# USNavalResearchLaboratory/mgen

Measured on AMD Instinct MI355X. Metric: device-resident MgenMsg pack+unpack GB/s and Mmsg/s at 1/2/4/8 MI355X, higher is better.
Workload: dtype u8; 1 GPU; udp_unpack_crc_1M_x_1024B; records_per_gpu=1048576, record_bytes=1024, checksum=True, output=mgenx_rec rows (32 B), parallelism=flow-sharded x1 (independent slabs)

## Files before the change

mgen_amd/csrc/mgenx_unpack.hip:

```cpp
#include <type_traits>

#include "mgenx_kernels.hpp"
#include "mgenx_parse.hpp"

namespace mgenx {

constexpr int kUnpackThreads = 1024;
constexpr int kRep = 32;
constexpr int kRepDwords = 4 * 256 * kRep;
constexpr int kSmallTabDwords = 1024;
constexpr int kFoldTabs = 6;
constexpr size_t kUnpackLdsBytes = (size_t)(kRepDwords + kFoldTabs * kSmallTabDwords) * 4u;


__device__ __forceinline__ uint32_t a64_s1(uint32_t lane) { return ((lane & 31u) << 2) | (1u << 16); }

typedef __attribute__((address_space(3))) uint32_t lds_u32_t;
__device__ __forceinline__ uint32_t lds_u32(const uint8_t*, uint32_t addr, uint32_t imm) {
  return *(const lds_u32_t*)(addr + imm);
}

__device__ __forceinline__ uint32_t xor3(uint32_t a, uint32_t b, uint32_t c) {
  return __builtin_amdgcn_bitop3_b32(a, b, c, 0x96);
}
// ... 1055 lines not shown
      st_g8_nt(at(u8b, 1), r.o[4]);
      return;
    }
    st_g32(at(u32, 4), r.o[0]);
    st_g32(at((uint64_t)c.dst_addr4, 4), r.o[1]);
    st_g16(at(u16, 2), r.o[2]);
    st_g8(at(u8a, 1), r.o[3]);
    st_g8(at(u8b, 1), r.o[4]);
  };
  auto decide = [&](const u32x4_t& pf, bool live) {
    const uint32_t w0 = prefix_word(pf, 0);
    const uint32_t w5 = prefix_word(pf, 5);
    const bool v2 = ((w0 >> 16) & 0xffu) == 2u;
    const bool flagged = force || ((((w0 >> 24) & MGENX_FLAG_CHECKSUM) != 0) && v2);
    const uint32_t t = (w5 >> 16) & 0xffu;
    return live && flagged && (tcp || (v2 && (t == 1u || t == 2u)));
  };

  u32x4_t pf;
  auto load_group = [&](uint32_t gg) {
    const uint32_t i = rec_idx(gg);
    const uint32_t boff = base_off(is_live(i), i);
    if (!kAligned) pf = ld_hdr(boff);
#pragma unroll
    for (int j = 0; j < NR; j++) {
      d[j] = ld_row(boff, j);
      __builtin_amdgcn_sched_barrier(0);
    }
  };
  load_group(g);
  table_writes(lds, tab_regs);
  asm volatile("s_waitcnt lgkmcnt(0)" ::: "memory");
  __builtin_amdgcn_s_barrier();
  if (g >= g_end) return;
  bool first = true;
  while (g < g_end) {
    uint32_t idx = rec_idx(g);
    bool live = is_live(idx);
    if (!first) {
      const uint32_t boff = base_off(live, idx);
      if (!kAligned) pf = ld_hdr(boff);
#pragma unroll
      for (int j = 0; j < NR; j++) {
        d[j] = ld_row(boff, j);
        __builtin_amdgcn_sched_barrier(0);
      }
    }
    first = false;
    auto step = [&](const u32x4_t& pf_cur, u32x4_t& pf_nxt) {
      const uint32_t gn = g + n_waves;
      const bool has_next = gn < g_end;
      const uint32_t idx_n = rec_idx(has_next ? gn : g);
      const bool live_n = has_next && is_live(idx_n);
      const uint32_t boff_n = base_off(live_n, idx_n);
      if (!kAligned) pf_nxt = ld_hdr(boff_n);
      asm volatile("" ::: "memory");
      const u32x4_t hdr = kAligned ? d[0] : pf_cur;
      const bool needs_crc = decide(hdr, live);
      const bool any = __any(needs_crc);
      Out early;
      if (kAligned && !kAblNoTail) early = decode(hdr, idx, live);

      uint32_t ha[4] = {0u, 0u, 0u, 0u}, hb[4] = {0u, 0u, 0u, 0u};
#pragma unroll
      for (int j = 0; j < NR - 1; j++) {
        u32x4_t x = d[j];
        if (j == 0) {
          const int s0 = -pos0;
          if (s0 > 0) {
            const u32x4_t zero = {0u, 0u, 0u, 0u};
            x = s0 < 16 ? shl_bytes(x, s0) : zero;
          }
        }
        const uint32_t xw[4] = {x.x, x.y, x.z, x.w};
        uint32_t c4[4];
#pragma unroll
        for (int b = 0; b < 4; b++) {
          if (kAblXor)
            c4[b] = (ha[b] << 1) ^ xw[b];
          else
            c4[b] = xor3(ha[b], hb[b], xw[b]);
        }
        __builtin_amdgcn_sched_barrier(0);
        d[j] = ld_row(boff_n, j);
        __builtin_amdgcn_sched_barrier(0);
        if (kAblXor) {
#pragma unroll
          for (int b = 0; b < 4; b++) ha[b] = c4[b];
          continue;
        }
#pragma unroll
        for (int b = 0; b < 4; b++) a64_parts(ldsb, c4[b], s1, ha[b], hb[b]);
      }
      const u32x4_t xf = d[NR - 1];
      uint32_t f0 = xor3(ha[0], hb[0], xf.x), f1 = xor3(ha[1], hb[1], xf.y);
      uint32_t f2 = xor3(ha[2], hb[2], xf.z);
      uint32_t f3 = xor3(ha[3], hb[3], q == 3 ? bswap32(xf.w) : xf.w);
      asm volatile("" : "+v"(f0), "+v"(f1), "+v"(f2), "+v"(f3));
      __builtin_amdgcn_sched_barrier(0);
      d[NR - 1] = ld_row(boff_n, NR - 1);
      __builtin_amdgcn_sched_barrier(0);
      const uint32_t v = shift_tab(fold + 3 * 1024, f0) ^ shift_tab(fold + 2 * 1024, f1) ^
                         shift_tab(fold + 1 * 1024, f2) ^ shift_tab(fold, f3);
      const uint32_t* lt = fold + (q == 0 ? 5 : (q == 1 ? 4 : 3)) * 1024;
      uint32_t s = (q == 3) ? v : shift_tab(lt, v);
      s ^= __shfl_xor(s, 1);
      s ^= __shfl_xor(s, 2);
      if (kAblNoTail) {
        if (s == 0x9E3779B9u && lane == 0) p.cols.err[idx] = (uint8_t)needs_crc;
      } else {
        const Out r = kAligned ? early : decode(hdr, idx, live);
        emit(r, idx, needs_crc && s != expect);
      }
      asm volatile("" ::"v"(boff_n + (uint32_t)(pos0 + 64)));
      g = gn;
      idx = idx_n;
      live = live_n;
      return has_next && any;
    };
    u32x4_t pf2;
    if (kAligned) {
      while (step(pf, pf2)) {
      }
    } else {
      for (;;) {
        if (!step(pf, pf2)) break;
        if (!step(pf2, pf)) break;
      }
    }
    for (; g < g_end; g += n_waves) {
      const uint32_t i = rec_idx(g);
      const bool lv = is_live(i);
      const u32x4_t ph = ld_hdr(base_off(lv, i));
      const bool nc = decide(ph, lv);
      if (__any(nc)) break;
      emit(decode(ph, i, lv), i, false);
    }
  }
  if (kAblBurst) {
    uint32_t k = 0;
    for (uint32_t gg = wave_id; gg < g_end; gg += n_waves, k++) {
      const uint32_t i = rec_idx(gg);
      const uint64_t seq = (uint64_t)wave_id * 8192u + k * 512u + 8u * (uint32_t)lane;
      const uint64_t a = (uint64_t)p.cols.rows + (kAblBurstSeq ? seq : (uint64_t)i * 32 + 8 * q);
      if (i < p.n) {
        if (kAblWt) st_g64_wt(a, (uint64_t)gg);
        else if (kAblAltStore) st_g64(a, (uint64_t)gg);
        else st_g64_nt(a, (uint64_t)gg);
      }
    }
  }
}

template <int NR, int RS = 4, int K = 16>
__global__ void __launch_bounds__(kUnpackThreads)
unpack_fixed_ring_kernel(UnpackParams p, uint32_t expect) {
  static_assert(NR == 8 || NR == 16, "ring kernel: 512- or 1024-byte records");
  static_assert(NR % RS == 0, "the ring divides the record's rows");
  extern __shared__ __attribute__((aligned(16))) uint32_t lds[];
  const uint32_t* fold = lds + kRepDwords;
  const uint8_t* ldsb = reinterpret_cast<const uint8_t*>(lds);
  const TableRegs tab_regs = table_loads(p.tabs);
  asm volatile("" ::: "memory");

  const int lane = threadIdx.x & 63;
  const int q = lane & 3;
  const uint32_t s1 = a64_s1((uint32_t)lane);
  const uint32_t wave_id = __builtin_amdgcn_readfirstlane(
      blockIdx.x * (blockDim.x >> 6) + (threadIdx.x >> 6));
  const uint32_t n_waves = gridDim.x * (blockDim.x >> 6);
  const uint32_t g_end = (p.n + 15u) >> 4;
  const bool force = (p.opts & MGENX_OPT_CHECKSUM_FORCE) != 0;
  const bool tcp = (p.opts & MGENX_OPT_TCP) != 0;
  const uint32_t L = p.fixed_len;

  auto rec_idx = [&](uint32_t gg) { return (gg << 4) + (uint32_t)(lane >> 2); };
  auto is_live = [&](uint32_t i) {
    const uint64_t off = (uint64_t)i * p.stride;
    return i < p.n && off <= p.slab_bytes && L <= p.slab_bytes - off;
  };
  auto row_base = [&](uint32_t gg) {
    const uint32_t i = rec_idx(gg);
    return (is_live(i) ? i * (uint32_t)p.stride : 64u) + 16u * (uint32_t)q;
  };
  auto ld = [&](uint32_t base, int j) { return ldu128(p.slab + (uint64_t)base + 64 * j); };
  auto decide = [&](const u32x4_t& pf, bool live) {
    const uint32_t w0 = prefix_word(pf, 0);
    const uint32_t w5 = prefix_word(pf, 5);
    const bool v2 = ((w0 >> 16) & 0xffu) == 2u;
    const bool flagged = force || ((((w0 >> 24) & MGENX_FLAG_CHECKSUM) != 0) && v2);
    const uint32_t t = (w5 >> 16) & 0xffu;
    return live && flagged && (tcp || (v2 && (t == 1u || t == 2u)));
  };
  auto decode = [&](const u32x4_t& pf, uint32_t idx, bool live, uint32_t& o0, uint32_t& o1) {
    uint32_t w[8];
#pragma unroll
    for (int j = 0; j < 8; j++) w[j] = prefix_word(pf, j);
    const uint32_t w10 = prefix_word(pf, 10);
    const uint32_t D = w[5] >> 24;
    const uint32_t hw = (D == 4u) ? w[7] : w10;
    const uint32_t gi = (28u + D + (hw >> 24)) >> 2;
    const uint32_t g3 = (prefix_word(pf, 11) & (0u - (uint32_t)(gi == 8u))) |
                        (prefix_word(pf, 12) & (0u - (uint32_t)(gi == 9u))) |
                        (prefix_word(pf, 14) & (0u - (uint32_t)(gi == 11u))) |
                        (prefix_word(pf, 15) & (0u - (uint32_t)(gi == 12u)));
    uint32_t flow = bswap32(w[1]), seq = bswap32(w[2]), sec = bswap32(w[3]);
    uint32_t usec = bswap32(w[4]), dst4 = w[6];
    uint32_t msg_len = bswap16((uint16_t)(w[0] & 0xffffu));
    uint32_t dport = bswap16((uint16_t)(w[5] & 0xffffu));
    const uint32_t hlen = 44u + D + (hw >> 24);
    uint32_t plen = bswap16((uint16_t)(g3 >> 16));
    if (!(plen != 0 && hlen + plen <= L)) plen = 0;
    uint32_t flags = w[0] >> 24, err = 0, dtype = (w[5] >> 16) & 0xffu, dlen = D;
    uint32_t ptype = (g3 >> 8) & 0xffu, gps = g3 & 0xffu;
    const bool slow = live && !fast_layout(w[0], w[5], hw);
    if (__any(slow)) {
      Hdr h;
      if (slow && q == 0) parse_header(p.slab + (uint64_t)idx * p.stride, L, false, w, h);
      auto bc = [&](uint32_t& dst, uint32_t v) {
        v = (uint32_t)__builtin_amdgcn_mov_dpp((int)v, 0x00, 0xf, 0xf, false);
        if (slow) dst = v;
      };
      bc(flow, h.flow); bc(seq, h.seq); bc(sec, h.sec); bc(usec, h.usec); bc(dst4, h.dst4);
      bc(msg_len, h.msg_len); bc(dport, h.dst_port); bc(plen, h.plen); bc(flags, h.flags);
      bc(err, h.err); bc(dtype, h.dst_type); bc(dlen, h.dst_len); bc(ptype, h.ptype);
      bc(gps, h.gps);
    }
    if (!live) {
      flow = seq = sec = usec = dst4 = msg_len = dport = plen = flags = dtype = dlen = 0;
      ptype = gps = 0;
      err = MGENX_ERROR_OOB;
    }
    o0 = q == 0 ? flow : q == 1 ? sec : q == 2 ? dst4 : (plen | flags << 16 | err << 24);
    o1 = q == 0 ? seq : q == 1 ? usec : q == 2 ? (msg_len | dport << 16)
                                              : (dtype | dlen << 8 | ptype << 16 | gps << 24);
  };
  auto verdict = [&](uint32_t& o0, bool crc_bad) {
    const uint32_t fl = tcp ? (uint32_t)MGENX_FLAG_CHECKSUM_ERROR : 0u;
    if (crc_bad && q == 3) o0 = (o0 & 0x00ffffffu) | fl << 16 | (uint32_t)MGENX_ERROR_CHECKSUM << 24;
  };

  uint32_t b0[K], b1[K];
#pragma unroll
  for (int k = 0; k < K; k++) b0[k] = b1[k] = 0u;
  uint32_t held = 0, last_g = 0;
  auto push = [&](uint32_t o0, uint32_t o1, uint32_t gg) {
#pragma unroll
    for (int k = 0; k < K - 1; k++) {
      b0[k] = b0[k + 1];
      b1[k] = b1[k + 1];
    }
    b0[K - 1] = o0;
    b1[K - 1] = o1;
    held++;
    last_g = gg;
  };
  auto flush = [&]() {
#pragma unroll
    for (int k = 0; k < K; k++) {
      const uint32_t back = (uint32_t)(K - 1 - k);
      const uint32_t gg = last_g - back * n_waves;
      const uint32_t idx = rec_idx(gg);
      const bool in = back < held && idx < p.n;
      const uint64_t v = (uint64_t)b1[k] << 32 | b0[k];
      if (back < held)
        st_g64_nt(in ? (uint64_t)p.cols.rows + (uint64_t)idx * 32 + 8 * q
                     : (uint64_t)p.sink + 8u * (uint32_t)lane, v);
    }
    held = 0;
  };

  u32x4_t d[RS];
  uint32_t g = wave_id;
  const uint32_t base0 = row_base(g < g_end ? g : 0u);
#pragma unroll
  for (int j = 0; j < RS; j++) {
    d[j] = ld(base0, j);
    __builtin_amdgcn_sched_barrier(0);
  }
  table_writes(lds, tab_regs);
  asm volatile("s_waitcnt lgkmcnt(0)" ::: "memory");
  __builtin_amdgcn_s_barrier();
  if (g >= g_end) return;

  bool pipelined = true;
  while (g < g_end) {
    const uint32_t gn = g + n_waves;
    const bool has_next = gn < g_end;
    const uint32_t idx = rec_idx(g);
    const bool live = is_live(idx);
    if (pipelined) {
      const uint32_t base = row_base(g), base_n = row_base(has_next ? gn : g);
      const u32x4_t hdr = d[0];
      const bool needs_crc = decide(hdr, live);
      const bool any = __any(needs_crc);
      uint32_t o0, o1;
      decode(hdr, idx, live, o0, o1);
      uint32_t ha[4] = {0u, 0u, 0u, 0u}, hb[4] = {0u, 0u, 0u, 0u};
#pragma unroll
      for (int j = 0; j < NR - 1; j++) {
        const u32x4_t x = d[j % RS];
        const uint32_t xw[4] = {x.x, x.y, x.z, x.w};
        uint32_t c4[4];
#pragma unroll
        for (int b = 0; b < 4; b++) c4[b] = xor3(ha[b], hb[b], xw[b]);
        __builtin_amdgcn_sched_barrier(0);
        d[j % RS] = (j + RS < NR) ? ld(base, j + RS) : ld(base_n, j + RS - NR);
        __builtin_amdgcn_sched_barrier(0);
#pragma unroll
        for (int b = 0; b < 4; b++) a64_parts(ldsb, c4[b], s1, ha[b], hb[b]);
      }
      const u32x4_t xf = d[(NR - 1) % RS];
      uint32_t f0 = xor3(ha[0], hb[0], xf.x), f1 = xor3(ha[1], hb[1], xf.y);
      uint32_t f2 = xor3(ha[2], hb[2], xf.z);
      uint32_t f3 = xor3(ha[3], hb[3], q == 3 ? bswap32(xf.w) : xf.w);
      asm volatile("" : "+v"(f0), "+v"(f1), "+v"(f2), "+v"(f3));
      __builtin_amdgcn_sched_barrier(0);
      d[(NR - 1) % RS] = ld(base_n, NR - 1 + RS - NR);
      __builtin_amdgcn_sched_barrier(0);
      const uint32_t v = shift_tab(fold + 3 * 1024, f0) ^ shift_tab(fold + 2 * 1024, f1) ^
                         shift_tab(fold + 1 * 1024, f2) ^ shift_tab(fold, f3);
      const uint32_t* lt = fold + (q == 0 ? 5 : (q == 1 ? 4 : 3)) * 1024;
      uint32_t sum = (q == 3) ? v : shift_tab(lt, v);
      sum ^= __shfl_xor(sum, 1);
      sum ^= __shfl_xor(sum, 2);
      verdict(o0, needs_crc && sum != expect);
      push(o0, o1, g);
      asm volatile("" ::"v"(base_n));
      pipelined = has_next && any;
    } else {
      const u32x4_t ph = ld(row_base(g), 0);
      if (__any(decide(ph, live))) {
        const uint32_t bb = row_base(g);
#pragma unroll
        for (int j = 0; j < RS; j++) d[j] = ld(bb, j);
        pipelined = true;
        continue;
      }
      uint32_t o0, o1;
      decode(ph, idx, live, o0, o1);
      push(o0, o1, g);
    }
    if (held == (uint32_t)K) flush();
    g = gn;
  }
  if (held) flush();
}

constexpr int kLongNB = 8;
constexpr uint32_t kLongMin = 4096;
constexpr int kLongFold = 7;
constexpr size_t kLongLdsBytes = (size_t)(kRepDwords + kLongFold * kSmallTabDwords) * 4u;
static_assert(kLongLdsBytes <= 160u * 1024u, "long-record tables fit the CU's LDS");

template <int NB = kLongNB, int NT = kUnpackThreads>
__global__ void __launch_bounds__(NT) unpack_long_kernel(UnpackParams p) {
  static_assert(1024 % NT == 0, "table staging: whole passes");
  extern __shared__ __attribute__((aligned(16))) uint32_t lds[];
  const uint32_t* fold = lds + kRepDwords;
  const uint32_t *fA4 = fold, *fA16 = fold + 1024, *fA32 = fold + 2048, *fA64 = fold + 3072,
                 *fA128 = fold + 4096, *fA256 = fold + 5120, *fA512 = fold + 6144;
  const uint8_t* ldsb = reinterpret_cast<const uint8_t*>(lds);
  constexpr int kFoldIdx[kLongFold] = {kTabA4, kTabA16, kTabA32, kTabA64, kTabA128, kTabA256,
                                       kTabA512};
  const uint32_t a1024 = p.tabs[kTabA1024 * 1024 + threadIdx.x];
  uint32_t fr[kLongFold];
#pragma unroll
  for (int k = 0; k < kLongFold; k++) fr[k] = p.tabs[kFoldIdx[k] * 1024 + threadIdx.x];
  constexpr int kNB = NB;

  const int lane = threadIdx.x & 63;
  const int q = lane & 3, quad = lane >> 2;
  const uint32_t s1 = a64_s1((uint32_t)lane);
  const uint32_t wave_id = __builtin_amdgcn_readfirstlane(
      blockIdx.x * (blockDim.x >> 6) + (threadIdx.x >> 6));
  const uint32_t n_waves = gridDim.x * (blockDim.x >> 6);
  const bool force = (p.opts & MGENX_OPT_CHECKSUM_FORCE) != 0;
  const bool tcp = (p.opts & MGENX_OPT_TCP) != 0;
  const bool want_ext = p.cols.dst_addr || p.cols.host_addr;
  const mgenx_cols& cc = p.cols;
  const bool any_ext = cc.hdr_len || cc.payload_off || cc.host_port || cc.host_type ||
                       cc.host_len || cc.lat_raw || cc.lon_raw || cc.alt || cc.dst_addr ||
                       cc.host_addr || cc.decoded;
  const uint8_t* dummy = reinterpret_cast<const uint8_t*>(p.tabs);

  struct Rec {
    uint32_t idx;
    uint64_t off;
    uint32_t L;
    bool live;
    bool rows;
    uint32_t nb;
    int64_t r0;
  };
  auto place = [&](uint32_t ri) {
    Rec r;
    r.idx = ri;
    r.off = 0;
    r.L = 0;
    if (ri < p.n) {
      r.off = p.rec_off ? p.rec_off[ri] : (uint64_t)ri * p.stride;
      r.L = p.rec_len ? p.rec_len[ri] : p.fixed_len;
    }
    const bool oob = ri < p.n && (r.L > 65535u || r.off > p.slab_bytes || r.L > p.slab_bytes - r.off);
    r.live = ri < p.n && !oob;
    r.rows = r.live && r.L >= 32u;
    const uint32_t R = r.rows ? (r.L + 1023u) >> 10 : 0u;
    r.nb = R ? (R + kNB - 1u) / kNB : 1u;
    r.r0 = (int64_t)(r.rows ? r.L : 0u) - 1024 * (int64_t)(kNB * r.nb);
    return r;
  };
  auto row_pos = [&](const Rec& r, uint32_t b, int j) {
    return r.r0 + 1024 * (int64_t)(kNB * b + (uint32_t)j) + 16 * lane;
  };
  auto ld_row = [&](const Rec& r, uint32_t b, int j) {
    const int64_t pos = row_pos(r, b, j);
    return ldu128(r.rows && pos >= 0 ? p.slab + r.off + (uint64_t)pos
                                     : (r.rows && pos > -16 ? p.slab + r.off : dummy));
  };

  Rec cur = place(wave_id);
  uint32_t b = 0;
  u32x4_t d[kNB];
#pragma unroll
  for (int j = 0; j < kNB; j++) {
    d[j] = ld_row(cur, 0, j);
    __builtin_amdgcn_sched_barrier(0);
  }
  {
    typedef __attribute__((address_space(3))) u32x4_t lds_u32x4_t;
    for (uint32_t e = threadIdx.x; e < 1024u; e += NT) {
      const uint32_t k = e >> 8, val = e & 255u;
      const uint32_t av = e == threadIdx.x ? a1024 : p.tabs[kTabA1024 * 1024 + e];
      const u32x4_t s = {av, av, av, av};
      lds_u32x4_t* dst = (lds_u32x4_t*)((k >> 1) * 65536u + val * 256u + (k & 1u) * 128u);
#pragma unroll
      for (int c = 0; c < kRep / 4; c++) dst[c] = s;
      uint32_t* fl = lds + kRepDwords;
#pragma unroll
      for (int k2 = 0; k2 < kLongFold; k2++)
        fl[k2 * 1024 + e] = e == threadIdx.x ? fr[k2] : p.tabs[kFoldIdx[k2] * 1024 + e];
    }
  }
  asm volatile("s_waitcnt lgkmcnt(0)" ::: "memory");
  __builtin_amdgcn_s_barrier();
  if (cur.idx >= p.n) return;

  uint32_t ha[4] = {0u, 0u, 0u, 0u}, hb[4] = {0u, 0u, 0u, 0u};
  u32x4_t pf = {0u, 0u, 0u, 0u}, xs = {0u, 0u, 0u, 0u};
  uint32_t expect = 0;
  auto start_record = [&](const Rec& r) {
    pf = ldu128((r.live && quad == 0 && r.L >= 16u * (q + 1)) ? p.slab + r.off + 16 * q : dummy);
    expect = p.expect[r.live ? r.L : 0u];
    const int s = (int)(16u - (r.L & 15u)) & 15;
    const u32x4_t x0 = ldu128(r.rows ? p.slab + r.off : dummy);
    xs = s ? shl_bytes(x0, s) : x0;
  };
  start_record(cur);
  while (true) {
    const bool last = b + 1u == cur.nb;
    const Rec nx = last ? place(cur.idx + n_waves) : cur;
    const uint32_t bn = last ? 0u : b + 1u;
    const bool has_next = nx.idx < p.n;
    const bool fix = cur.r0 + 1024 * (int64_t)(kNB * b) < 0;
    u32x4_t xf = {0u, 0u, 0u, 0u};
#pragma unroll
    for (int j = 0; j < kNB; j++) {
      u32x4_t x = d[j];
      if (fix) {
        const int64_t pos = row_pos(cur, b, j);
        const bool zero = pos <= -16, strad = pos < 0 && pos > -16;
        x.x = zero ? 0u : (strad ? xs.x : x.x);
        x.y = zero ? 0u : (strad ? xs.y : x.y);
        x.z = zero ? 0u : (strad ? xs.z : x.z);
        x.w = zero ? 0u : (strad ? xs.w : x.w);
      }
      if (last && j == kNB - 1) {
        uint32_t f0 = xor3(ha[0], hb[0], x.x), f1 = xor3(ha[1], hb[1], x.y);
        uint32_t f2 = xor3(ha[2], hb[2], x.z);
        uint32_t f3 = xor3(ha[3], hb[3], lane == 63 ? bswap32(x.w) : x.w);
        asm volatile("" : "+v"(f0), "+v"(f1), "+v"(f2), "+v"(f3));
        xf = u32x4_t{f0, f1, f2, f3};
        __builtin_amdgcn_sched_barrier(0);
        d[j] = has_next ? ld_row(nx, bn, j) : ldu128(dummy);
        __builtin_amdgcn_sched_barrier(0);
      } else {
        const uint32_t xw[4] = {x.x, x.y, x.z, x.w};
        uint32_t c4[4];
#pragma unroll
        for (int k = 0; k < 4; k++) c4[k] = xor3(ha[k], hb[k], xw[k]);
        __builtin_amdgcn_sched_barrier(0);
        d[j] = has_next ? ld_row(nx, bn, j) : ldu128(dummy);
        __builtin_amdgcn_sched_barrier(0);
#pragma unroll
        for (int k = 0; k < 4; k++) a64_parts(ldsb, c4[k], s1, ha[k], hb[k]);
      }
    }
    if (last) {
      uint32_t v = shift_tab(fA4, xf.x) ^ xf.y;
      v = shift_tab(fA4, v) ^ xf.z;
      v = shift_tab(fA4, v) ^ xf.w;
      v = shift_tab(fA4, v);
      v = (q & 1) ? v : shift_tab(fA16, v);
      v ^= __shfl_xor(v, 1);
      v = (q & 2) ? v : shift_tab(fA32, v);
      v ^= __shfl_xor(v, 2);
      v = (quad & 1) ? v : shift_tab(fA64, v);
      v ^= __shfl_xor(v, 4);
      v = (quad & 2) ? v : shift_tab(fA128, v);
      v ^= __shfl_xor(v, 8);
      v = (quad & 4) ? v : shift_tab(fA256, v);
      v ^= __shfl_xor(v, 16);
      v = (quad & 8) ? v : shift_tab(fA512, v);
      v ^= __shfl_xor(v, 32);
      const uint32_t tot = v;
      const uint32_t L = cur.L;
      const bool live = cur.live;
      const uint8_t* rec = p.slab + cur.off;
      const uint32_t buf_len = tcp ? min(L, (uint32_t)MGENX_TX_BUFFER_SIZE) : L;
      uint32_t pw[16];
      quad_bcast<0>(pf, pw);
      quad_bcast<1>(pf, pw);
      quad_bcast<2>(pf, pw);
      quad_bcast<3>(pf, pw);
      if (lane == 0) {
        if (live) {
          uint32_t w[8];
          const bool pfx = L >= 32;
          if (pfx) {
#pragma unroll
            for (int j = 0; j < 8; j++) w[j] = pw[j];
          } else if (L >= MGENX_MIN_SIZE) {
            load_fixed(rec, buf_len, w);
          } else {
#pragma unroll
            for (int j = 0; j < 8; j++) w[j] = 0;
          }
          const bool flagged = force || (((w[0] >> 24) & MGENX_FLAG_CHECKSUM) != 0 &&
                                         buf_len >= MGENX_MIN_SIZE && ((w[0] >> 16) & 0xffu) == 2u);
          const bool needs_crc = flagged && (tcp ? (L >= 4) : fixed_ok(buf_len, w));
          const bool crc_ok = !needs_crc || (cur.rows ? tot == expect : small_crc_ok(rec, L));
          if (buf_len >= 64 && fast_layout(pw[0], pw[5], (pw[5] >> 24) == 4u ? pw[7] : pw[10])) {
            store_fast_q0(p.cols, cur.idx, pw, buf_len, crc_ok, tcp);
            if (any_ext) store_fast_ext(p.cols, cur.idx, [&](int k) { return pw[k]; }, buf_len, true);
          } else {
            Hdr h;
            parse_header(rec, buf_len, want_ext, w, h);
            store_hdr_q0(p.cols, cur.idx, h, crc_ok, tcp);
          }
        } else {
          store_oob_q0(p.cols, cur.idx);
        }
      }
#pragma unroll
      for (int k = 0; k < 4; k++) ha[k] = hb[k] = 0u;
      if (!has_next) break;
      start_record(nx);
    }
    cur = nx;
    b = bn;
  }
}

template <typename K>
static hipError_t launch_lds(K kernel, const UnpackParams& p, int grid, hipStream_t stream) {
  hipError_t e = set_max_lds((const void*)kernel, (int)kUnpackLdsBytes);
  if (e != hipSuccess) return e;
  hipLaunchKernelGGL(kernel, dim3(grid), dim3(kUnpackThreads), kUnpackLdsBytes, stream, p);
  return hipGetLastError();
}

template <int MODE>
static hipError_t launch_mode(const UnpackParams& p, int grid, hipStream_t stream) {
  return launch_lds(unpack_kernel<true, MODE>, p, grid, stream);
}

template <int NT = kUnpackThreads, int KB = 4, int MODE = 0>
static hipError_t launch_var(const UnpackParams& p, int grid, hipStream_t stream) {
  hipError_t e = set_max_lds((const void*)unpack_var_kernel<NT, KB, MODE>, (int)kUnpackLdsBytes);
  if (e != hipSuccess) return e;
  hipLaunchKernelGGL((unpack_var_kernel<NT, KB, MODE>), dim3(grid), dim3(NT), kUnpackLdsBytes,
                     stream, p);
  return hipGetLastError();
}

template <int NB = kLongNB, int NT = kUnpackThreads>
static hipError_t launch_long_t(const UnpackParams& p, int grid, hipStream_t stream) {
  hipError_t e = set_max_lds((const void*)unpack_long_kernel<NB, NT>, (int)kLongLdsBytes);
  if (e != hipSuccess) return e;
  hipLaunchKernelGGL((unpack_long_kernel<NB, NT>), dim3(grid), dim3(NT), kLongLdsBytes, stream, p);
  return hipGetLastError();
}
static hipError_t launch_long(const UnpackParams& p, int grid, hipStream_t stream) {
#if MGENX_DIAG
  switch (p.variant) {
    case 40: return launch_long_t<16, 512>(p, grid, stream);
    case 41: return launch_long_t<8, 512>(p, grid, stream);
    case 42: return launch_long_t<4, 1024>(p, grid, stream);
    case 43: return launch_long_t<12, 512>(p, grid, stream);
    case 44: return launch_long_t<2, 1024>(p, grid, stream);
    case 45: return launch_long_t<16, 1024>(p, grid, stream);
    default: break;
  }
#endif
  return launch_long_t<>(p, grid, stream);
}

#if MGENX_DIAG
static hipError_t launch_sorted(const UnpackParams& p, int grid, hipStream_t stream) {
  return launch_lds(unpack_kernel<true, 0, true>, p, grid, stream);
}
#endif

template <int NR, int MODE = 0, bool kRows = false, bool kAligned = false>
static hipError_t launch_fixed(const UnpackParams& p, int grid, hipStream_t stream) {
  hipError_t e = set_max_lds((const void*)unpack_fixed_kernel<NR, MODE, kRows, kAligned>, (int)kUnpackLdsBytes);
  if (e != hipSuccess) return e;
  hipLaunchKernelGGL((unpack_fixed_kernel<NR, MODE, kRows, kAligned>), dim3(grid),
                     dim3(kUnpackThreads), kUnpackLdsBytes, stream, p, p.expect_fixed);
  return hipGetLastError();
}

template <int NR, int RS = 4, int K = 16>
static hipError_t launch_ring(const UnpackParams& p, int grid, hipStream_t stream) {
  hipError_t e = set_max_lds((const void*)unpack_fixed_ring_kernel<NR, RS, K>, (int)kUnpackLdsBytes);
  if (e != hipSuccess) return e;
  hipLaunchKernelGGL((unpack_fixed_ring_kernel<NR, RS, K>), dim3(grid), dim3(kUnpackThreads),
                     kUnpackLdsBytes, stream, p, p.expect_fixed);
  return hipGetLastError();
}

typedef hipError_t (*fixed_launcher)(const UnpackParams&, int, hipStream_t);
#define MGENX_FIXED_TABLE(R)                                                              \
  {nullptr, nullptr, launch_fixed<2, 0, R>, launch_fixed<3, 0, R>, launch_fixed<4, 0, R>,    \
   launch_fixed<5, 0, R>, launch_fixed<6, 0, R>, launch_fixed<7, 0, R>, launch_fixed<8, 0, R>, \
   launch_fixed<9, 0, R>, launch_fixed<10, 0, R>, launch_fixed<11, 0, R>,                    \
   launch_fixed<12, 0, R>, launch_fixed<13, 0, R>, launch_fixed<14, 0, R>,                   \
   launch_fixed<15, 0, R>, launch_fixed<16, 0, R>}
static const fixed_launcher kFixedLaunch[17] = MGENX_FIXED_TABLE(false);
static const fixed_launcher kFixedLaunchRows[17] = MGENX_FIXED_TABLE(true);
#undef MGENX_FIXED_TABLE

hipError_t launch_unpack(const UnpackParams& p, int grid, hipStream_t stream, int* which) {
  const int unpack_variant = p.variant;
  *which = MGENX_UNPACK_K_OTHER;
  if (p.opts & MGENX_OPT_SKIP_CRC) {
    *which = MGENX_UNPACK_K_HEADER;
    hipLaunchKernelGGL((unpack_kernel<false>), dim3(grid), dim3(kUnpackThreads), 0, stream, p);
    return hipGetLastError();
  }
  const mgenx_cols& c = p.cols;
  const bool ext = c.hdr_len || c.payload_off || c.host_port || c.host_type || c.host_len ||
                   c.lat_raw || c.lon_raw || c.alt || c.dst_addr || c.host_addr || c.decoded;
  const uint32_t nr = (p.fixed_len + 63) / 64;
  const bool fixed = !p.rec_off && !p.rec_len && p.fixed_len >= 65 && p.fixed_len <= 1024 &&
                     p.stride > 0 && p.n <= 0xFFFFFFF0u && !ext &&
                     p.slab_bytes < 0xFFFF0000ull && p.slab_bytes >= 64ull * (nr + 1) + 16 &&
                     p.slab_bytes >= p.fixed_len;
  if (unpack_variant == 0 && fixed) {
    *which = (c.rows && (p.fixed_len == 512 || p.fixed_len == 1024)) ? MGENX_UNPACK_K_FIXED_RING
                                                                    : MGENX_UNPACK_K_FIXED;
    switch (p.fixed_len) {
      case 256: return c.rows ? launch_fixed<4, 0, true, true>(p, grid, stream)
                              : launch_fixed<4, 0, false, true>(p, grid, stream);
      case 512: return c.rows ? launch_ring<8>(p, grid, stream)
                              : launch_fixed<8, 0, false, true>(p, grid, stream);
      case 1024: return c.rows ? launch_ring<16>(p, grid, stream)
                               : launch_fixed<16, 0, false, true>(p, grid, stream);
      default: break;
    }
    return (c.rows ? kFixedLaunchRows : kFixedLaunch)[(p.fixed_len + 63) / 64](p, grid, stream);
  }
#if MGENX_DIAG
  if (unpack_variant == 13 && fixed && p.fixed_len == 1024)
    return c.rows ? launch_fixed<16, 0, true, true>(p, grid, stream)
                  : launch_fixed<16, 0, false, true>(p, grid, stream);
  if (unpack_variant >= 14 && unpack_variant <= 16 && fixed && p.fixed_len == 1024 && c.rows) {
    if (unpack_variant == 14) return launch_ring<16, 8, 12>(p, grid, stream);
    if (unpack_variant == 15) return launch_ring<16, 8, 8>(p, grid, stream);
    return launch_ring<16, 4, 12>(p, grid, stream);
  }
  if (unpack_variant == 12 && fixed && p.fixed_len == 1024)
    return c.rows ? launch_fixed<16, 0, true>(p, grid, stream) : launch_fixed<16, 0>(p, grid, stream);
  if (unpack_variant >= 1024 && fixed && p.fixed_len == 1024) {
    switch (unpack_variant - 1024) {
#define MGENX_ABL(M) \
  case M: return c.rows ? launch_fixed<16, M, true, true>(p, grid, stream) \
                        : launch_fixed<16, M, false, true>(p, grid, stream);
      MGENX_ABL(1) MGENX_ABL(2) MGENX_ABL(3) MGENX_ABL(4) MGENX_ABL(5) MGENX_ABL(8)
      MGENX_ABL(16) MGENX_ABL(32) MGENX_ABL(64)
      MGENX_ABL(128) MGENX_ABL(144) MGENX_ABL(130) MGENX_ABL(136) MGENX_ABL(260) MGENX_ABL(772)
      MGENX_ABL(276) MGENX_ABL(324) MGENX_ABL(788)
#undef MGENX_ABL
      default: break;
    }
  }
  switch (unpack_variant) {
    case 1: return launch_mode<1>(p, grid, stream);
    case 2: return launch_mode<2>(p, grid, stream);
    case 3: return launch_mode<0>(p, grid, stream);
    case 4: return launch_sorted(p, grid, stream);
    default: break;
  }
  if (p.rec_len && unpack_variant >= 20 && unpack_variant < 40) {
    *which = MGENX_UNPACK_K_VAR;
    switch (unpack_variant) {
      case 20: return launch_var<1024, 0, 1>(p, grid, stream);
      case 21: return launch_var<1024, 0, 0>(p, grid, stream);
      case 22: return launch_var<768, 8, 0>(p, grid, stream);
      case 23: return launch_var<768, 16, 0>(p, grid, stream);
      case 27: return launch_var<1024, 8, 0>(p, grid, stream);
      case 32: return launch_var<1024, 4, 8>(p, grid, stream);
      case 33: return launch_var<1024, 4, 16>(p, grid, stream);
      default: break;
    }
  }
#endif
  const uint64_t mean = p.rec_len ? (p.n ? p.slab_bytes / p.n : 0) : p.fixed_len;
  if (mean >= kLongMin) {
    *which = MGENX_UNPACK_K_LONG;
    return launch_long(p, grid, stream);
  }
  const uint64_t tiles = ((uint64_t)p.n + 63) / 64;
  const uint64_t waves = (uint64_t)grid * (kUnpackThreads / 64);
  if (p.rec_len && tiles >= 2 * waves) {
    *which = MGENX_UNPACK_K_VAR;
    return launch_var(p, grid, stream);
  }
  *which = MGENX_UNPACK_K_GENERAL;
  return launch_mode<0>(p, grid, stream);
}

#if MGENX_DIAG
__global__ void __launch_bounds__(256) stream_read_kernel(const u32x4_t* p, uint64_t n16,
                                                          uint32_t* out) {
  uint32_t acc = 0;
  const uint64_t stride = (uint64_t)gridDim.x * blockDim.x;
  uint64_t i = (uint64_t)blockIdx.x * blockDim.x + threadIdx.x;
  for (; i + 3 * stride < n16; i += 4 * stride) {
    const u32x4_t a = p[i], b = p[i + stride], c = p[i + 2 * stride], d = p[i + 3 * stride];
    acc ^= a.x ^ a.y ^ a.z ^ a.w ^ b.x ^ b.y ^ b.z ^ b.w ^ c.x ^ c.y ^ c.z ^ c.w ^ d.x ^ d.y ^
           d.z ^ d.w;
  }
  for (; i < n16; i += stride) {
    const u32x4_t a = p[i];
    acc ^= a.x ^ a.y ^ a.z ^ a.w;
  }
  if (acc == 0x9E3779B9u) out[blockIdx.x] = acc;
}

template <int MODE>
__global__ void __launch_bounds__(1024) group_rw_kernel(const uint8_t* p, uint32_t n_groups,
                                                        uint8_t* out) {
  const int lane = threadIdx.x & 63;
  const uint32_t wave_id = __builtin_amdgcn_readfirstlane(blockIdx.x * 16 + (threadIdx.x >> 6));
  const uint32_t n_waves = gridDim.x * 16;
  uint32_t g = wave_id;
  if (g >= n_groups) return;
  const uint32_t lo = (uint32_t)(lane >> 2) * 1024u + 16u * (lane & 3);
  u32x4_t d[16];
#pragma unroll
  for (int j = 0; j < 16; j++) d[j] = ldu128(p + (uint64_t)g * 16384u + lo + 64 * j);
  uint32_t acc = 0;
  while (g < n_groups) {
    const uint32_t gn = g + n_waves;
    const uint32_t gl = gn < n_groups ? gn : g;
#pragma unroll
    for (int j = 0; j < 16; j++) {
      acc = (acc << 1) ^ d[j].x ^ d[j].y ^ d[j].z ^ d[j].w;
      __builtin_amdgcn_sched_barrier(0);
      d[j] = ldu128(p + (uint64_t)gl * 16384u + lo + 64 * j);
      __builtin_amdgcn_sched_barrier(0);
    }
    if (MODE & 4) {
      if (lane < 32) {
        u32x4_t v = {acc, g, acc, g};
        *reinterpret_cast<u32x4_t*>(out + (uint64_t)g * 512u + 16u * lane) = v;
      }
    } else if (MODE & 1) {
      const uint64_t a = (uint64_t)out + (uint64_t)g * 512u + 8u * lane;
      const uint64_t v = (uint64_t)acc << 32 | g;
      if (MODE & 2) st_g64_wt(a, v); else st_g64(a, v);
    }
    g = gn;
  }
  if (!(MODE & 1) && acc == 0x9E3779B9u) out[lane] = 1;
}

template <int LK, int POL>
__global__ void __launch_bounds__(1024) group_rw_buf_kernel(const uint8_t* p, uint32_t n_groups,
                                                            uint8_t* out) {
  constexpr int K = 1 << LK;
  const int lane = threadIdx.x & 63;
  const uint32_t wave_id = __builtin_amdgcn_readfirstlane(blockIdx.x * 16 + (threadIdx.x >> 6));
  const uint32_t n_waves = gridDim.x * 16;
  uint32_t g = wave_id;
  if (g >= n_groups) return;
  const uint32_t lo = (uint32_t)(lane >> 2) * 1024u + 16u * (lane & 3);
  u32x4_t d[16];
#pragma unroll
  for (int j = 0; j < 16; j++) d[j] = ldu128(p + (uint64_t)g * 16384u + lo + 64 * j);
  uint32_t acc = 0;
  while (g < n_groups) {
    uint64_t buf[K];
    uint32_t gs[K];
#pragma unroll
    for (int k = 0; k < K; k++) {
      const uint32_t gn = g + n_waves;
      const uint32_t gl = gn < n_groups ? gn : g;
#pragma unroll
      for (int j = 0; j < 16; j++) {
        acc = (acc << 1) ^ d[j].x ^ d[j].y ^ d[j].z ^ d[j].w;
        __builtin_amdgcn_sched_barrier(0);
        d[j] = ldu128(p + (uint64_t)gl * 16384u + lo + 64 * j);
        __builtin_amdgcn_sched_barrier(0);
      }
      buf[k] = (uint64_t)acc << 32 | g;
      gs[k] = g;
      g = gn;
    }
#pragma unroll
    for (int k = 0; k < K; k++) {
      const uint64_t a = (uint64_t)out + (uint64_t)(gs[k] < n_groups ? gs[k] : 0u) * 512u + 8u * lane;
      if (POL == 0) st_g64_nt(a, buf[k]);
      else if (POL == 1) st_g64(a, buf[k]);
      else st_g64_wt(a, buf[k]);
    }
  }
}

template <int RING, bool BAR, int POL>
__global__ void __launch_bounds__(1024) group_rw_phase_kernel(const uint8_t* p, uint32_t n_groups,
                                                              uint8_t* out, uint32_t* counter) {
// ... 139 lines not shown
```

Measured before the change: 5733 GB/s.

## Route column-output unpack through ring kernel with blocked group scheduling

The ring kernel gains a columnar-output flush that uses DPP lane shuffles to scatter decoded fields into the per-field column arrays, and it now replaces the fixed kernel for 512/1024-byte records when rows output is absent. Group scheduling becomes blocked: each wave walks 2^bshift consecutive groups before striding, and per-group ids are kept in a lane vector read back with readlane. The rows path keeps max_b=1, so it stays effectively strided, though its flush now derives indices through readlane. This workload writes rows, so the main changes there are the readlane index path and next_group bookkeeping overhead.

```diff
diff --git a/mgen_amd/csrc/mgenx_unpack.hip b/mgen_amd/csrc/mgenx_unpack.hip
--- a/mgen_amd/csrc/mgenx_unpack.hip
+++ b/mgen_amd/csrc/mgenx_unpack.hip
@@ -1231,9 +1231,9 @@
   }
 }
 
-template <int NR, int RS = 4, int K = 16>
+template <int NR, int RS = 4, int K = 16, bool kCols = false>
 __global__ void __launch_bounds__(kUnpackThreads)
-unpack_fixed_ring_kernel(UnpackParams p, uint32_t expect) {
+unpack_fixed_ring_kernel(UnpackParams p, uint32_t expect, uint32_t bshift) {
   static_assert(NR == 8 || NR == 16, "ring kernel: 512- or 1024-byte records");
   static_assert(NR % RS == 0, "the ring divides the record's rows");
   extern __shared__ __attribute__((aligned(16))) uint32_t lds[];
@@ -1319,10 +1319,11 @@
     if (crc_bad && q == 3) o0 = (o0 & 0x00ffffffu) | fl << 16 | (uint32_t)MGENX_ERROR_CHECKSUM << 24;
   };
 
+  static_assert(K <= 64, "one lane of gidv per held group");
   uint32_t b0[K], b1[K];
 #pragma unroll
   for (int k = 0; k < K; k++) b0[k] = b1[k] = 0u;
-  uint32_t held = 0, last_g = 0;
+  uint32_t held = 0, gidv = 0;
   auto push = [&](uint32_t o0, uint32_t o1, uint32_t gg) {
 #pragma unroll
     for (int k = 0; k < K - 1; k++) {
@@ -1331,27 +1332,94 @@
     }
     b0[K - 1] = o0;
     b1[K - 1] = o1;
+    gidv = (uint32_t)lane == held ? gg : gidv;
     held++;
-    last_g = gg;
   };
   auto flush = [&]() {
-#pragma unroll
-    for (int k = 0; k < K; k++) {
-      const uint32_t back = (uint32_t)(K - 1 - k);
-      const uint32_t gg = last_g - back * n_waves;
-      const uint32_t idx = rec_idx(gg);
-      const bool in = back < held && idx < p.n;
-      const uint64_t v = (uint64_t)b1[k] << 32 | b0[k];
-      if (back < held)
-        st_g64_nt(in ? (uint64_t)p.cols.rows + (uint64_t)idx * 32 + 8 * q
-                     : (uint64_t)p.sink + 8u * (uint32_t)lane, v);
-    }
+    const uint64_t sink = (uint64_t)p.sink + 8u * (uint32_t)lane;
+    const uint32_t r = (uint32_t)(lane >> 2);
+    const int q_lane = q;
+    auto gid = [&](int k) {
+      return (uint32_t)__builtin_amdgcn_readlane((int)gidv, (int)(((uint32_t)k + held - (uint32_t)K) & 63u));
+    };
+    if (!kCols) {
+#pragma unroll
+      for (int k = 0; k < K; k++) {
+        if ((uint32_t)(K - 1 - k) < held) {
+          const uint32_t idx = (gid(k) << 4) + r;
+          const uint64_t v = (uint64_t)b1[k] << 32 | b0[k];
+          st_g64_nt(idx < p.n ? (uint64_t)p.cols.rows + (uint64_t)idx * 32 + 8 * q : sink, v);
+        }
+      }
+      held = 0;
+      return;
+    }
+#define MGENX_QDPP(V, CTRL) ((uint32_t)__builtin_amdgcn_mov_dpp((int)(V), CTRL, 0xf, 0xf, false))
+    const mgenx_cols& c = p.cols;
+    int q = q_lane;
+    asm volatile("" : "+v"(q));
+    const uint32_t odd = 0u - (uint32_t)(q & 1), hi2 = 0u - (uint32_t)(q >> 1);
+    auto each = [&](uint64_t base, uint32_t size, auto value, auto store) {
+      __builtin_amdgcn_sched_barrier(0);
+      const uint64_t a = base + (uint64_t)(r * size);
+#pragma unroll
+      for (int k = 0; k < K; k++) {
+        if ((uint32_t)(K - 1 - k) < held) {
+          const uint32_t gk = gid(k);
+          const uint32_t v = value(b0[k], b1[k]);
+          store((gk << 4) + r < p.n ? a + (uint64_t)gk * (16u * size) : sink, v);
+        }
+      }
+    };
+    each(pick4(q, (uint64_t)c.flow_id, (uint64_t)c.seq_num, (uint64_t)c.tx_sec, (uint64_t)c.tx_usec),
+         4, [&](uint32_t x0, uint32_t x1) {
+           const uint32_t lo = MGENX_QDPP(x0, 0x50), hi = MGENX_QDPP(x1, 0x50);
+           return (lo & ~odd) | (hi & odd);
+         }, [](uint64_t a, uint32_t v) { st_g32(a, v); });
+    each((uint64_t)c.dst_addr4, 4, [&](uint32_t x0, uint32_t) { return MGENX_QDPP(x0, 0xAA); },
+         [](uint64_t a, uint32_t v) { st_g32(a, v); });
+    each(pick4(q, (uint64_t)c.msg_len, (uint64_t)c.dst_port, (uint64_t)c.payload_len,
+               (uint64_t)c.payload_len),
+         2, [&](uint32_t x0, uint32_t x1) {
+           const uint32_t md = MGENX_QDPP(x1, 0xAA), pl = MGENX_QDPP(x0, 0xFF);
+           return (((md >> (q == 1 ? 16 : 0)) & ~hi2) | (pl & hi2)) & 0xffffu;
+         }, [](uint64_t a, uint32_t v) { st_g16(a, v); });
+    each(pick4(q, (uint64_t)c.flags, (uint64_t)c.err, (uint64_t)c.dst_type, (uint64_t)c.dst_len),
+         1, [&](uint32_t x0, uint32_t x1) {
+           const uint32_t fe = MGENX_QDPP(x0, 0xFF), td = MGENX_QDPP(x1, 0xFF);
+           return (((fe >> (q == 1 ? 24 : 16)) & ~hi2) | ((td >> (q == 3 ? 8 : 0)) & hi2)) & 0xffu;
+         }, [](uint64_t a, uint32_t v) { st_g8(a, v); });
+    each(pick4(q, (uint64_t)c.payload_type, (uint64_t)c.gps_status, (uint64_t)c.payload_type,
+               (uint64_t)c.gps_status),
+         1, [&](uint32_t, uint32_t x1) {
+           const uint32_t td = MGENX_QDPP(x1, 0xFF);
+           return (td >> ((q & 1) ? 24 : 16)) & 0xffu;
+         }, [](uint64_t a, uint32_t v) { st_g8(a, v); });
+#undef MGENX_QDPP
     held = 0;
   };
 
+  constexpr uint32_t kNoGroup = 0xFFFFFFFFu;
+  const uint32_t bmask = (1u << bshift) - 1u;
+  auto next_group = [&](uint32_t& bk, uint32_t& tt) {
+    for (;;) {
+      if (tt == bmask) {
+        tt = 0;
+        bk += n_waves;
+      } else {
+        tt++;
+      }
+      const uint32_t first = bk << bshift;
+      if (first >= g_end) return kNoGroup;
+      const uint32_t gg = first + ((wave_id + tt) & bmask);
+      if (gg < g_end) return gg;
+    }
+  };
+  uint32_t blk = wave_id - n_waves, bt = bmask;
+
   u32x4_t d[RS];
-  uint32_t g = wave_id;
-  const uint32_t base0 = row_base(g < g_end ? g : 0u);
+  uint32_t g = next_group(blk, bt);
+  const uint32_t base0 = row_base(g != kNoGroup ? g : 0u);
 #pragma unroll
   for (int j = 0; j < RS; j++) {
     d[j] = ld(base0, j);
@@ -1360,12 +1428,13 @@
   table_writes(lds, tab_regs);
   asm volatile("s_waitcnt lgkmcnt(0)" ::: "memory");
   __builtin_amdgcn_s_barrier();
-  if (g >= g_end) return;
+  if (g == kNoGroup) return;
 
   bool pipelined = true;
-  while (g < g_end) {
-    const uint32_t gn = g + n_waves;
-    const bool has_next = gn < g_end;
+  while (g != kNoGroup) {
+    uint32_t blk_n = blk, bt_n = bt;
+    const uint32_t gn = next_group(blk_n, bt_n);
+    const bool has_next = gn != kNoGroup;
     const uint32_t idx = rec_idx(g);
     const bool live = is_live(idx);
     if (pipelined) {
@@ -1422,6 +1491,8 @@
     }
     if (held == (uint32_t)K) flush();
     g = gn;
+    blk = blk_n;
+    bt = bt_n;
   }
   if (held) flush();
 }
@@ -1700,14 +1771,23 @@
   return hipGetLastError();
 }
 
-template <int NR, int RS = 4, int K = 16>
-static hipError_t launch_ring(const UnpackParams& p, int grid, hipStream_t stream) {
-  hipError_t e = set_max_lds((const void*)unpack_fixed_ring_kernel<NR, RS, K>, (int)kUnpackLdsBytes);
+template <int NR, int RS = 4, int K = 16, bool kCols = false>
+static hipError_t launch_ring(const UnpackParams& p, int grid, hipStream_t stream, uint32_t max_b) {
+  hipError_t e = set_max_lds((const void*)unpack_fixed_ring_kernel<NR, RS, K, kCols>,
+                             (int)kUnpackLdsBytes);
   if (e != hipSuccess) return e;
-  hipLaunchKernelGGL((unpack_fixed_ring_kernel<NR, RS, K>), dim3(grid), dim3(kUnpackThreads),
-                     kUnpackLdsBytes, stream, p, p.expect_fixed);
+  const uint64_t groups = ((uint64_t)p.n + 15) / 16;
+  const uint64_t waves = (uint64_t)grid * (kUnpackThreads / 64);
+  if (max_b > (uint32_t)K) max_b = K;
+  uint32_t bshift = 0;
+  while ((2u << bshift) <= max_b && ((uint64_t)(2u << bshift)) * waves <= groups) bshift++;
+  hipLaunchKernelGGL((unpack_fixed_ring_kernel<NR, RS, K, kCols>), dim3(grid),
+                     dim3(kUnpackThreads), kUnpackLdsBytes, stream, p, p.expect_fixed, bshift);
   return hipGetLastError();
 }
+
+constexpr uint32_t kRingRowsMaxB = 1;
+constexpr uint32_t kRingColsMaxB = 2;
 
 typedef hipError_t (*fixed_launcher)(const UnpackParams&, int, hipStream_t);
 #define MGENX_FIXED_TABLE(R)                                                              \
@@ -1737,15 +1817,15 @@
                      p.slab_bytes < 0xFFFF0000ull && p.slab_bytes >= 64ull * (nr + 1) + 16 &&
                      p.slab_bytes >= p.fixed_len;
   if (unpack_variant == 0 && fixed) {
-    *which = (c.rows && (p.fixed_len == 512 || p.fixed_len == 1024)) ? MGENX_UNPACK_K_FIXED_RING
-                                                                    : MGENX_UNPACK_K_FIXED;
+    *which = (p.fixed_len == 512 || p.fixed_len == 1024) ? MGENX_UNPACK_K_FIXED_RING
+                                                         : MGENX_UNPACK_K_FIXED;
     switch (p.fixed_len) {
       case 256: return c.rows ? launch_fixed<4, 0, true, true>(p, grid, stream)
                               : launch_fixed<4, 0, false, true>(p, grid, stream);
-      case 512: return c.rows ? launch_ring<8>(p, grid, stream)
-                              : launch_fixed<8, 0, false, true>(p, grid, stream);
-      case 1024: return c.rows ? launch_ring<16>(p, grid, stream)
-                               : launch_fixed<16, 0, false, true>(p, grid, stream);
+      case 512: return c.rows ? launch_ring<8>(p, grid, stream, kRingRowsMaxB)
+                              : launch_ring<8, 4, 16, true>(p, grid, stream, kRingColsMaxB);
+      case 1024: return c.rows ? launch_ring<16>(p, grid, stream, kRingRowsMaxB)
+                               : launch_ring<16, 4, 16, true>(p, grid, stream, kRingColsMaxB);
       default: break;
     }
     return (c.rows ? kFixedLaunchRows : kFixedLaunch)[(p.fixed_len + 63) / 64](p, grid, stream);
@@ -1755,9 +1835,19 @@
     return c.rows ? launch_fixed<16, 0, true, true>(p, grid, stream)
                   : launch_fixed<16, 0, false, true>(p, grid, stream);
   if (unpack_variant >= 14 && unpack_variant <= 16 && fixed && p.fixed_len == 1024 && c.rows) {
-    if (unpack_variant == 14) return launch_ring<16, 8, 12>(p, grid, stream);
-    if (unpack_variant == 15) return launch_ring<16, 8, 8>(p, grid, stream);
-    return launch_ring<16, 4, 12>(p, grid, stream);
+    if (unpack_variant == 14) return launch_ring<16, 8, 12>(p, grid, stream, kRingRowsMaxB);
+    if (unpack_variant == 15) return launch_ring<16, 8, 8>(p, grid, stream, kRingRowsMaxB);
+    return launch_ring<16, 4, 12>(p, grid, stream, kRingRowsMaxB);
+  }
+  if (unpack_variant >= 17 && unpack_variant <= 21 && fixed &&
+      (p.fixed_len == 512 || p.fixed_len == 1024)) {
+    const uint32_t max_b = 1u << (unpack_variant - 17);
+    *which = MGENX_UNPACK_K_FIXED_RING;
+    if (p.fixed_len == 512)
+      return c.rows ? launch_ring<8>(p, grid, stream, max_b)
+                    : launch_ring<8, 4, 16, true>(p, grid, stream, max_b);
+    return c.rows ? launch_ring<16>(p, grid, stream, max_b)
+                  : launch_ring<16, 4, 16, true>(p, grid, stream, max_b);
   }
   if (unpack_variant == 12 && fixed && p.fixed_len == 1024)
     return c.rows ? launch_fixed<16, 0, true>(p, grid, stream) : launch_fixed<16, 0>(p, grid, stream);
```

Result: no change. 5742 GB/s, median of 6 (+0.2%).
